# DJT777/xlstm-yolo-clean

Hardware: NVIDIA B200
Metric: mLSTM chunkwise fwd+bwd TFLOP/s (algorithmic, 14*L*d*(L+d) per chunk) (higher is better)
Workload: dtype bf16

## Files before the change

### xlstm_yolo_clean_b200/csrc/tensor_kernels.cu

```cuda
#include <atomic>
#include <mutex>
#include <set>
#include <type_traits>
#include <utility>

#include "common.cuh"
#include "sm100.cuh"

namespace mlstm {
namespace {

using namespace sm100;

constexpr int LT = 128;
constexpr int kWorkers = 256;
constexpr int kTcThreads = 320;
constexpr int kCtlWarp = 8, kScanWarp = 9;
constexpr int kNbAB = kWorkers + 32;
constexpr int kNbC = kWorkers + 64;
constexpr float kLog2e = 1.4426950408889634f;
enum { NB_A = 1, NB_B = 2, NB_C = 3, NB_PAIR0 = 4 };

struct GateBuf {
  static constexpr int oB = 0, oI = LT, oPm = 2 * LT, oY = 3 * LT, oF = 4 * LT, oMt = 5 * LT, oNt = 6 * LT,
// ... 1041 lines not shown
        for (int u = ch; u < 4; u += 2) {
          float v[32];
          const bool off_diag = REV ? u > rb : u < rb;
          if (off_diag) {
            tmem_ld32(tS + lane_base + u * 32, v);
            const float r_t = ex2_approx(x_t + gb[GateBuf::oScal + 4 + u]);
#pragma unroll
            for (int j4 = 0; j4 < 8; ++j4) {
              const float4 cf = *reinterpret_cast<const float4*>(scf + u * 32 + 4 * j4);
              v[4 * j4 + 0] *= cf.x * r_t;
              v[4 * j4 + 1] *= cf.y * r_t;
              v[4 * j4 + 2] *= cf.z * r_t;
              v[4 * j4 + 3] *= cf.w * r_t;
              rs += (v[4 * j4 + 0] + v[4 * j4 + 1]) + (v[4 * j4 + 2] + v[4 * j4 + 3]);
            }
          } else if (u == rb) {
            tmem_ld32(tS + lane_base + u * 32, v);
#pragma unroll
            for (int j4 = 0; j4 < 8; ++j4) {
              const float4 y = *reinterpret_cast<const float4*>(sy + u * 32 + 4 * j4);
              const float yy[4] = {y.x, y.y, y.z, y.w};
#pragma unroll
              for (int e = 0; e < 4; ++e) {
                const int j = 4 * j4 + e;
                float pv = v[j] * ex2_approx(x_t + yy[e]);
                pv = (REV ? j >= lane : j <= lane) ? pv : 0.f;
                rs += pv;
                v[j] = pv;
              }
            }
          } else {
#pragma unroll
            for (int j = 0; j < 32; ++j) v[j] = 0.f;
          }
          store_row32<T>(sP, row, u * 32, v);
        }
        srs[ch * LT + row] = rs;
      }
      fence_proxy_async_smem();
      tc_fence_before_sync();
      named_arrive(NB_B, kNbAB);
      {
        const float ab = __expf(g - b_t + i_t - m_next);
#pragma unroll 1
        for (int hf = 0; hf < 2; ++hf) {
          float kb[32];
#pragma unroll
          for (int j = 0; j < 4; ++j) {
            uint4 u = *reinterpret_cast<const uint4*>(sK + ch * SM::kTile + swz128(row, hf * 32 + 8 * j));
            float2 a0 = unpack2<T>(u.x), a1 = unpack2<T>(u.y), a2 = unpack2<T>(u.z), a3 = unpack2<T>(u.w);
            kb[8 * j + 0] = a0.x * ab; kb[8 * j + 1] = a0.y * ab; kb[8 * j + 2] = a1.x * ab; kb[8 * j + 3] = a1.y * ab;
            kb[8 * j + 4] = a2.x * ab; kb[8 * j + 5] = a2.y * ab; kb[8 * j + 6] = a3.x * ab; kb[8 * j + 7] = a3.y * ab;
          }
          store_row32<T>(sKb, row, ch * 64 + hf * 32, kb);
          const float cs = warp_colsum32(kb, lane);
          snp[rb * D + ch * 64 + hf * 32 + lane] = cs;
        }
        fence_proxy_async_smem();
        named_arrive(NB_A, kNbAB);
      }
      mbar_wait(&bar_h, par, 7);
      tc_fence_after_sync();
      {
        const float bq = __expf(b_t + m_run - m_t) * p.scale;
        const float den = bq * (sqn[row] + sqn[LT + row]) + srs[row] + srs[LT + row];
        const float nmax = fmaxf(fabsf(den), __expf(-m_t));
        const float inv = p.sig == 2 ? 1.f : 1.f / (nmax + p.eps);
#pragma unroll 1
        for (int hf = 0; hf < 2; ++hf) {
          uint32_t hi[32], hx[32];
          tmem_ld32_nowait(tHi + lane_base + ch * 64 + hf * 32, hi);
          tmem_ld32_nowait(tHx + lane_base + ch * 64 + hf * 32, hx);
          tmem_ld_wait();
          float o[32];
#pragma unroll
          for (int j = 0; j < 32; ++j) o[j] = (__uint_as_float(hi[j]) + bq * __uint_as_float(hx[j])) * inv;
          store_row32<T>(sH, row, ch * 64 + hf * 32, o);
        }
        if (ch == 0 && row < n_valid) {
          p.n_out[(int64_t)bh * p.S + t0 + row] = nmax;
          p.m_out[(int64_t)bh * p.S + t0 + row] = m_t;
        }
        if (EPI) {
          uint8_t* sub = sH + ch * SM::kTile;
          const int64_t tok = (int64_t)(t0 + row);
          if (p.h_plain && row < n_valid) {
            uint4* dst = reinterpret_cast<uint4*>((T*)p.h_plain + b * p.h_sb + hh * p.h_sh + tok * p.h_ss + ch * 64);
#pragma unroll
            for (int j = 0; j < 8; ++j) dst[j] = *reinterpret_cast<const uint4*>(sub + swz128(row, 8 * j));
          }
          const void* xrow = p.x ? (const void*)((const uint16_t*)p.x + b * p.x_sb + hh * p.x_sh + tok * p.x_ss + ch * 64) : nullptr;
          ln_epilogue_slice<T, 128, 64>(sub, [](int r, int cc) { return swz128(r, cc & 63); }, row, ch * 64, ch, NB_PAIR0 + rb,
                                        fsm + SM::fStat, fsm + SM::fPar, xrow, p.xy_f16 != 0, p.ln_eps, row < n_valid);
        }
      }
      mbar_wait(&bar_dc, par, 6);
      tc_fence_after_sync();
      {
#pragma unroll
        for (int hf = 0; hf < 2; ++hf) {
          float v[32], t32[32];
          tmem_ld32(tDC + lane_base + ch * 64 + hf * 32, v);
#pragma unroll
          for (int j = 0; j < 32; ++j) {
            Creg[hf * 32 + j] = gbar * Creg[hf * 32 + j] + v[j];
            t32[j] = Creg[hf * 32 + j];
          }
          store_row32<T>(sC, row, ch * 64 + hf * 32, t32);
        }
        if (tid < D) {
          sNn[tid] = gbar * sNc[tid] + ((snp[tid] + snp[D + tid]) + (snp[2 * D + tid] + snp[3 * D + tid]));
          mbar_arrive(&bar_n);
        }
      }
      fence_proxy_async_smem();
      tc_fence_before_sync();
      named_arrive(NB_C, kNbC);
      m_run = m_next;
      cur ^= 1;
    }
    if (p.c_last) {
      float* dst = p.c_last + ((int64_t)bh * D + row) * D + ch * 64;
#pragma unroll
      for (int j = 0; j < 64; ++j) dst[j] = Creg[j];
      if (tid < D) p.n_last[(int64_t)bh * D + tid] = fsm[SM::fN + cur * D + tid];
      if (tid == 0) p.m_last[bh] = m_run;
    }
  }
  tc_fence_before_sync();
  __syncthreads();
  if (warp == kCtlWarp) tmem_dealloc<512>(tmem);
}

struct TcBwParams {
  int B, NH, S, NT;
  float eps, scale;
  const void *ig, *fg;
  int64_t ig_sb, ig_sh, ig_ss, fg_sb, fg_sh, fg_ss;
  const float* m0;
  const float *n_out, *m_out, *dc_last;
  void *di, *df;
  int64_t di_sb, di_sh, di_ss, df_sb, df_sh, df_ss;
  float* dc0;
  int rev;
  int sig;
  float cap;
  int acc_qk, acc_v, acc_g;
  int cs_rows, cs_off;
#ifdef MLSTM_TC_PROFILE
  long long* prof;
#endif
};

template <int D_>
struct BwSmem {
  static constexpr int D = D_;
  static constexpr int kTile = Lay<D>::kTile;
  static constexpr int kPTile = LT * 128;
  static constexpr int kState = Lay<D>::kState;
  static constexpr int kNST = D == 64 ? 1 : 2;
  static constexpr int kStage = 4 * kTile + kState;
  static constexpr int oQ = 0, oK = kTile, oV = 2 * kTile, odH = 3 * kTile, oCs = 4 * kTile;
  static constexpr int oQt = kNST * kStage;
  static constexpr int oSb = oQt + kTile;
  static constexpr int odS = oSb + 2 * kPTile;
  static constexpr int odQ = odS + 2 * kPTile;
  static constexpr int odV = odQ + kTile;
  static constexpr int odK = odV + kTile;
  static constexpr int odC = odK + kTile;
  static constexpr int oSmall = odC + kState;
  static constexpr int fGates = 0, fPart = 2 * GateBuf::kFloats, kSmallFloats = fPart + 12 * LT;
  static constexpr int kBytes = oSmall + kSmallFloats * 4 + 1024;
  static constexpr uint32_t kLoadBytes = 4 * kTile + kState;
  static constexpr bool kAlias = D == 64;
  static constexpr uint32_t cS = 0, cdSb = 128;
  static constexpr uint32_t cdV1 = D == 64 ? 0 : 256, cdV2 = cdV1 + D, cdK1 = D == 64 ? 128 : 320, cdK2 = cdK1 + D,
                            cdQa = D == 64 ? 256 : 384, cdQb = cdQa + D, cddC = D == 64 ? 384 : 448;
};

template <typename T, int D, bool REV, typename TO>
__global__ void __launch_bounds__(kTcThreads, 1)
tc_bw(const __grid_constant__ CUtensorMap mapQ, const __grid_constant__ CUtensorMap mapK,
          const __grid_constant__ CUtensorMap mapV, const __grid_constant__ CUtensorMap mapdH,
          const __grid_constant__ CUtensorMap mapCs, const __grid_constant__ CUtensorMap mapdQ,
          const __grid_constant__ CUtensorMap mapdK, const __grid_constant__ CUtensorMap mapdV, TcBwParams p) {
  constexpr bool kBf16 = std::is_same<T, __nv_bfloat16>::value;
  using SM = BwSmem<D>;
  using L = Lay<D>;
  constexpr int CW = L::CW;
  TC_PROF(200, 0);
  TC_PROF_CTA(0);
  extern __shared__ uint8_t smem_raw[];
  uint8_t* smem = smem_raw + ((1024u - (smem_u32(smem_raw) & 1023u)) & 1023u);
  uint8_t* sQ = smem + SM::oQ;
  uint8_t* sK = smem + SM::oK;
  uint8_t* sV = smem + SM::oV;
  uint8_t* sdH = smem + SM::odH;
  uint8_t* sQt = smem + SM::oQt;
  uint8_t* sSb = smem + SM::oSb;
  uint8_t* sdS = smem + SM::odS;
  uint8_t* sdQ = smem + SM::odQ;
  uint8_t* sdV = smem + SM::odV;
  uint8_t* sdK = smem + SM::odK;
  uint8_t* sCs = smem + SM::oCs;
  uint8_t* sdC = smem + SM::odC;
  float* fsm = (float*)(smem + SM::oSmall);
  __shared__ uint64_t bar_full[SM::kNST], bar_s, bar_q, bar_v, bar_k, bar_d, bar_b, bar_st, bar_g[2];
  __shared__ uint32_t tmem_base_s;

  const int tid = threadIdx.x, lane = tid & 31;
  const int warp = __shfl_sync(0xffffffffu, tid >> 5, 0);
  const int bh = blockIdx.x, b = bh / p.NH, hh = bh % p.NH;

  auto mt = [&](int c) { return REV ? p.NT - 1 - c : c; };
  auto load_stage = [&](int s, int c) {
    uint8_t* base = smem + s * SM::kStage;
    mbar_expect_tx(&bar_full[s], SM::kLoadBytes);
    tma_load_4d(base + SM::oQ, &mapQ, &bar_full[s], 0, mt(c) * LT, hh, b);
    tma_load_4d(base + SM::oK, &mapK, &bar_full[s], 0, mt(c) * LT, hh, b);
    tma_load_4d(base + SM::oV, &mapV, &bar_full[s], 0, mt(c) * LT, hh, b);
    tma_load_4d(base + SM::odH, &mapdH, &bar_full[s], 0, mt(c) * LT, hh, b);
    tma_load_4d(base + SM::oCs, &mapCs, &bar_full[s], 0, mt(c) * p.cs_rows + p.cs_off, hh, b);
  };
  if (tid == kCtlWarp * 32) {
    for (int s = 0; s < SM::kNST; ++s) mbar_init(&bar_full[s], 1);
    fence_mbar_init();
    grid_dep_wait();
    for (int s = 0; s < SM::kNST && s < p.NT; ++s) load_stage(s, p.NT - 1 - s);
  }
  if (tid == 0) {
    mbar_init(&bar_s, 1);
    mbar_init(&bar_b, 1);
    mbar_init(&bar_st, 1);
    mbar_init(&bar_q, 1);
    mbar_init(&bar_v, 1);
    mbar_init(&bar_k, 1);
    mbar_init(&bar_d, 1);
    mbar_init(&bar_g[0], 1);
    mbar_init(&bar_g[1], 1);
    fence_mbar_init();
  }
  if (warp == kCtlWarp) {
    tmem_alloc<512>(&tmem_base_s);
    if (lane == 0) {
      prefetch_tmap(&mapQ); prefetch_tmap(&mapK); prefetch_tmap(&mapV); prefetch_tmap(&mapdH);
      prefetch_tmap(&mapCs); prefetch_tmap(&mapdQ); prefetch_tmap(&mapdK); prefetch_tmap(&mapdV);
    }
  }
  grid_dep_wait();
  grid_dep_launch();
  const int rb = warp & 3, ch = (warp >> 2) & 1;
  const int row = rb * 32 + lane;
  const uint32_t lane_base = (uint32_t)(rb * 32) << 16;
  const int drow = rb * 16 + (lane & 15);
  const bool owns_c = warp < kCtlWarp && lane < 16 && rb * 16 < D;
  float dCreg[CW];
#pragma unroll
  for (int j = 0; j < CW; ++j) dCreg[j] = 0.f;
  if (warp < kCtlWarp) {
    if (p.dc_last && owns_c) {
      const float* src = p.dc_last + ((int64_t)bh * D + drow) * D + ch * CW;
#pragma unroll
      for (int j = 0; j < CW; ++j) dCreg[j] = src[j];
    }
    if (owns_c) store_cols<T, D>(sdC, drow, ch * CW, dCreg);
    fence_proxy_async_smem();
  }
  tc_fence_before_sync();
  __syncthreads();
  tc_fence_after_sync();
  const uint32_t tmem = tmem_base_s;
  const uint32_t tS = tmem + SM::cS, tdSb = tmem + SM::cdSb;
  const uint32_t tdV1 = tmem + SM::cdV1, tdV2 = tmem + SM::cdV2, tdK1 = tmem + SM::cdK1, tdK2 = tmem + SM::cdK2;
  const uint32_t tdQa = tmem + SM::cdQa, tdQb = tmem + SM::cdQb, tddC = tmem + SM::cddC;

  const T* ip = (const T*)p.ig + b * p.ig_sb + hh * p.ig_sh;
  const T* fp = (const T*)p.fg + b * p.fg_sb + hh * p.fg_sh;
  const float* mo = p.m_out + (int64_t)bh * p.S;
  const float* no = p.n_out + (int64_t)bh * p.S;
  if (warp == kCtlWarp) {
    constexpr uint32_t id_s = umma_idesc(128, 128, false, false, kBf16);
    constexpr uint32_t id_c = umma_idesc(64, D, true, true, kBf16);
    constexpr uint32_t id_k_mn = umma_idesc(128, D, false, true, kBf16);
    constexpr uint32_t id_mn_mn = umma_idesc(128, D, true, true, kBf16);
    constexpr uint32_t id_k_k = umma_idesc(128, D, false, false, kBf16);
    const uint64_t kQ0 = L::desc(smem_u32(sQ), 0), mQ0 = L::desc(smem_u32(sQ), SM::kTile);
    const uint64_t kK0 = L::desc(smem_u32(sK), 0), mK0 = L::desc(smem_u32(sK), SM::kTile);
    const uint64_t kV0 = L::desc(smem_u32(sV), 0);
    const uint64_t kH0 = L::desc(smem_u32(sdH), 0), mH0 = L::desc(smem_u32(sdH), SM::kTile);
    const uint64_t kCs0 = L::desc(smem_u32(sCs), 0);
    const uint64_t mQt = L::desc(smem_u32(sQt), D == 64 ? SM::kTile : 0);
    const uint64_t mSb = umma_smem_desc(smem_u32(sSb), SM::kPTile, 1024);
    const uint64_t kdS = umma_smem_desc(smem_u32(sdS), 0, 1024), mdS = umma_smem_desc(smem_u32(sdS), SM::kPTile, 1024);
    const uint64_t kdC = L::desc(smem_u32(sdC), 0), mdC = L::desc(smem_u32(sdC), SM::kState);
    auto issue_s = [&](int it) {
      const int s = it % SM::kNST;
      const uint32_t so = (uint32_t)s * SM::kStage;
      const uint64_t kQ = umma_desc_advance(kQ0, so), kK = umma_desc_advance(kK0, so);
      const uint64_t kH = umma_desc_advance(kH0, so), kV = umma_desc_advance(kV0, so);
      mbar_wait(&bar_full[s], (it / SM::kNST) & 1, 11);
      tc_fence_after_sync();
#pragma unroll
      for (int kk = 0; kk < D / 16; ++kk)
        umma_f16(tS, umma_desc_advance(kQ, kk * 32), umma_desc_advance(kK, kk * 32), id_s, kk > 0);
#pragma unroll
      for (int kk = 0; kk < D / 16; ++kk)
        umma_f16(tdSb, umma_desc_advance(kH, kk * 32), umma_desc_advance(kV, kk * 32), id_s, kk > 0);
      umma_commit(&bar_s);
    };

    if (elect_one()) issue_s(0);
    __syncwarp();

    for (int it = 0; it < p.NT; ++it) {
      const int c = p.NT - 1 - it, pb = it & 1;
      const uint32_t par = it & 1;
      const int t0 = mt(c) * LT, n_valid = min(LT, p.S - t0);
      const uint32_t so = (uint32_t)(it % SM::kNST) * SM::kStage;
      const uint64_t kQ = umma_desc_advance(kQ0, so), mQ = umma_desc_advance(mQ0, so);
      const uint64_t kK = umma_desc_advance(kK0, so), mK = umma_desc_advance(mK0, so);
      const uint64_t kV = umma_desc_advance(kV0, so), kCs = umma_desc_advance(kCs0, so);
      const uint64_t kH = umma_desc_advance(kH0, so), mH = umma_desc_advance(mH0, so);
      TC_PROF(it, 9);
      if (SM::kNST == 1 && c > 0 && lane == 0) {
        const int r = mt(c - 1) * LT;
        tma_prefetch_4d(&mapQ, 0, r, hh, b);
        tma_prefetch_4d(&mapK, 0, r, hh, b);
        tma_prefetch_4d(&mapV, 0, r, hh, b);
        tma_prefetch_4d(&mapdH, 0, r, hh, b);
        tma_prefetch_4d(&mapCs, 0, mt(c - 1) * p.cs_rows + p.cs_off, hh, b);
      }
      named_sync(NB_B, kNbAB);
      TC_PROF(it, 10);
      if (elect_one()) {
        tc_fence_after_sync();
#pragma unroll
        for (int kk = 0; kk < LT / 16; ++kk)
          umma_f16(tdK1, umma_desc_advance(mdS, kk * 2048), umma_desc_advance(mQ, kk * L::kAdvMN), id_mn_mn, kk > 0);
#pragma unroll
        for (int kk = 0; kk < D / 16; ++kk)
          umma_f16(tdK2, umma_desc_advance(kV, kk * 32), umma_desc_advance(kdC, kk * 32), id_k_k, kk > 0);
        umma_commit(&bar_k);
#pragma unroll
        for (int kk = 0; kk < LT / 16; ++kk)
          umma_f16(tdQa, umma_desc_advance(kdS, (kk / 4) * SM::kPTile + (kk % 4) * 32), umma_desc_advance(mK, kk * L::kAdvMN),
                   id_k_mn, kk > 0);
#pragma unroll
        for (int kk = 0; kk < D / 16; ++kk)
          umma_f16(tdQb, umma_desc_advance(kH, kk * 32), umma_desc_advance(kCs, kk * 32), id_k_k, kk > 0);
        umma_commit(&bar_q);
#pragma unroll
        for (int kk = 0; kk < D / 16; ++kk)
          umma_f16(tdV2, umma_desc_advance(kK, kk * 32), umma_desc_advance(mdC, kk * L::kAdvMN), id_k_mn, kk > 0);
        umma_commit(&bar_b);
      }
      __syncwarp();
      if (lane == 0) {
        tma_store_wait_read<0>();
        mbar_arrive(&bar_st);
      }
      __syncwarp();
      TC_PROF(it, 11);
      named_sync(NB_A, kNbAB);
      TC_PROF(it, 12);
      if (elect_one()) {
#pragma unroll
        for (int kk = 0; kk < LT / 16; ++kk)
          umma_f16(tddC, umma_desc_advance(mQt, kk * L::kAdvMN), umma_desc_advance(mH, kk * L::kAdvMN), id_c, kk > 0);
        umma_commit(&bar_d);
#pragma unroll
        for (int kk = 0; kk < LT / 16; ++kk)
          umma_f16(tdV1, umma_desc_advance(mSb, kk * 2048), umma_desc_advance(mH, kk * L::kAdvMN), id_mn_mn, kk > 0);
        umma_commit(&bar_v);
        if (!SM::kAlias && c > 0) issue_s(it + 1);
        if (SM::kNST == 1) {
          if (c > 0) {
            const int r = mt(c - 1) * LT;
            mbar_expect_tx(&bar_full[0], SM::kLoadBytes);
            mbar_wait(&bar_k, par, 21);
            tma_load_4d(sQ, &mapQ, &bar_full[0], 0, r, hh, b);
            tma_load_4d(sV, &mapV, &bar_full[0], 0, r, hh, b);
            mbar_wait(&bar_q, par, 24);
            tma_load_4d(sCs, &mapCs, &bar_full[0], 0, mt(c - 1) * p.cs_rows + p.cs_off, hh, b);
            mbar_wait(&bar_b, par, 22);
            tma_load_4d(sK, &mapK, &bar_full[0], 0, r, hh, b);
            mbar_wait(&bar_v, par, 25);
            tma_load_4d(sdH, &mapdH, &bar_full[0], 0, r, hh, b);
          }
        } else if (c >= SM::kNST) {
          mbar_wait(&bar_v, par, 25);
          load_stage(it % SM::kNST, c - SM::kNST);
        }
      }
      __syncwarp();
      TC_PROF(it, 13);
      named_sync(NB_C, kNbC);
      TC_PROF(it, 14);
      if (lane == 0) {
        if (p.acc_qk) {
          tma_reduce_add_4d(&mapdQ, sdQ, 0, t0, hh, b);
          tma_reduce_add_4d(&mapdK, sdK, 0, t0, hh, b);
        } else {
          tma_store_4d(&mapdQ, sdQ, 0, t0, hh, b);
          tma_store_4d(&mapdK, sdK, 0, t0, hh, b);
        }
        if (p.acc_v) tma_reduce_add_4d(&mapdV, sdV, 0, t0, hh, b);
        else tma_store_4d(&mapdV, sdV, 0, t0, hh, b);
        tma_store_commit();
      }
      __syncwarp();
      if (SM::kAlias && c > 0 && elect_one()) issue_s(it + 1);
      __syncwarp();
    }
    if (lane == 0) tma_store_wait_all<0>();
  } else if (warp == kScanWarp) {
    struct TileRaw {
      GateRaw<T> g;
      float4 mt, nt;
      float m_prev, m_next;
    };
    auto raw_of = [&](int c) {
      TileRaw r;
      const int t0 = mt(c) * LT, n_valid = min(LT, p.S - t0);
      r.g = load_gate_raw<T>(ip + (int64_t)t0 * p.ig_ss, p.ig_ss, fp + (int64_t)t0 * p.fg_ss, p.fg_ss, n_valid);
      if (lane * 4 < n_valid) {
        r.mt = *reinterpret_cast<const float4*>(mo + t0 + lane * 4);
        r.nt = p.sig == 2 ? make_float4(1.f, 1.f, 1.f, 1.f) : *reinterpret_cast<const float4*>(no + t0 + lane * 4);
      } else {
        r.mt = make_float4(0.f, 0.f, 0.f, 0.f);
        r.nt = make_float4(1.f, 1.f, 1.f, 1.f);
      }
      if (!REV) {
        r.m_prev = c > 0 ? mo[t0 - 1] : (p.m0 ? p.m0[bh] : 0.f);
        r.m_next = mo[t0 + n_valid - 1];
      } else {
        r.m_prev = c > 0 ? mo[t0 + LT] : (p.m0 ? p.m0[bh] : 0.f);
        r.m_next = mo[t0];
      }
      return r;
    };
    auto publish = [&](float* gb, const TileRaw& r) {
      gate_scan_regs(gb, r.g, REV, p.sig != 0, p.cap);
      reinterpret_cast<float4*>(gb + GateBuf::oMt)[lane] = r.mt;
      reinterpret_cast<float4*>(gb + GateBuf::oNt)[lane] = r.nt;
      if (lane == 0) {
        gb[GateBuf::oScal + 2] = r.m_prev;
        gb[GateBuf::oScal + 3] = r.m_next;
      }
    };

    TileRaw raw = raw_of(p.NT - 1);
    float carry = 0.f;
    for (int n = 0; n < p.NT + 2; ++n) {
      if (n >= 2) {
      const int it = n - 2;
      const int c = p.NT - 1 - it, pb = it & 1;
      const int t0 = mt(c) * LT, n_valid = min(LT, p.S - t0);
      named_sync(NB_C, kNbC);
      {
        const float* sp = fsm + SM::fPart + pb * 6 * LT;
        const float* gb = fsm + SM::fGates + pb * GateBuf::kFloats;
        float acc[4], di[4];
#pragma unroll
        for (int e = 0; e < 4; ++e) {
          const int t = lane * 4 + e;
          acc[e] = (sp[0 * LT + t] + sp[1 * LT + t]) - (sp[2 * LT + t] + sp[3 * LT + t]);
          di[e] = sp[4 * LT + t] + sp[5 * LT + t];
        }
        float incl, own;
        if (!REV) {
          acc[2] += acc[3];
          acc[1] += acc[2];
          acc[0] += acc[1];
          incl = own = acc[0];
#pragma unroll
          for (int o = 1; o < 32; o <<= 1) {
            float u = __shfl_down_sync(0xffffffffu, incl, o);
            if (lane + o < 32) incl += u;
          }
        } else {
          acc[1] += acc[0];
          acc[2] += acc[1];
          acc[3] += acc[2];
          incl = own = acc[3];
#pragma unroll
          for (int o = 1; o < 32; o <<= 1) {
            float u = __shfl_up_sync(0xffffffffu, incl, o);
            if (lane >= o) incl += u;
          }
        }
        const float excl = incl - own + carry;
        TO* dip = (TO*)p.di + b * p.di_sb + hh * p.di_sh;
        TO* dfp = (TO*)p.df + b * p.df_sb + hh * p.df_sh;
#pragma unroll
        for (int e = 0; e < 4; ++e) {
          const int t = lane * 4 + e;
          if (t < n_valid) {
            const float dsig = p.sig ? 1.f - __expf(gb[GateBuf::oI + t]) : 1.f;
            float gi = di[e] * dsig * gb[GateBuf::oDi + t];
            float gf = (acc[e] + excl) * sigmoid_neg_f32(gb[GateBuf::oF + t]) * gb[GateBuf::oDf + t];
            TO* pi = dip + (int64_t)(t0 + t) * p.di_ss;
            TO* pf = dfp + (int64_t)(t0 + t) * p.df_ss;
            if (p.acc_g) {
              gi += to_f32<TO>(*pi);
              gf += to_f32<TO>(*pf);
            }
            *pi = from_f32<TO>(gi);
            *pf = from_f32<TO>(gf);
          }
        }
        carry += __shfl_sync(0xffffffffu, incl, REV ? 31 : 0);
      }
      __syncwarp();
      }
      if (n < p.NT) {
        publish(fsm + SM::fGates + (n & 1) * GateBuf::kFloats, raw);
        __syncwarp();
        if (lane == 0) mbar_arrive(&bar_g[n & 1]);
        if (n + 1 < p.NT) raw = raw_of(p.NT - 2 - n);
      }
    }
  } else {
    for (int it = 0; it < p.NT; ++it) {
      const int pb = it & 1;
      const uint32_t par = it & 1;
      const float* gb = fsm + SM::fGates + pb * GateBuf::kFloats;
      float* spart = fsm + SM::fPart + pb * 6 * LT;
      const int n_valid = min(LT, p.S - mt(p.NT - 1 - it) * LT);
      const bool valid = row < n_valid;
      const uint32_t so = (uint32_t)(it % SM::kNST) * SM::kStage;

      TC_PROF(it, 0);
      mbar_wait(&bar_g[pb], (it >> 1) & 1, 12);
      const float g = gb[GateBuf::oScal], m_prev = gb[GateBuf::oScal + 2], m_next = gb[GateBuf::oScal + 3];
      const float b_t = gb[GateBuf::oB + row], i_t = gb[GateBuf::oI + row];
      const float m_t = gb[GateBuf::oMt + row], n_t = gb[GateBuf::oNt + row];
      const float rinv = !valid ? 0.f : p.sig == 2 ? 1.f : 1.f / (n_t + p.eps);
      const float bbar = valid ? __expf(b_t + m_prev - m_t) : 0.f;
      const float abar = __expf(g - b_t + i_t - m_next);
      const float gbar = __expf(g + m_prev - m_next);
      TC_PROF(it, 1);
      mbar_wait(&bar_full[it % SM::kNST], (it / SM::kNST) & 1, 13);
      uint32_t qs[CW / 2];
      {
        const float wq = p.scale * bbar * rinv;
#pragma unroll
        for (int j = 0; j < CW / 8; ++j) {
          const uint32_t off = L::swz(row, ch * CW + 8 * j);
          uint4 u = *reinterpret_cast<const uint4*>(sQ + so + off);
          qs[4 * j] = u.x; qs[4 * j + 1] = u.y; qs[4 * j + 2] = u.z; qs[4 * j + 3] = u.w;
          float2 a0 = unpack2<T>(u.x), a1 = unpack2<T>(u.y), a2 = unpack2<T>(u.z), a3 = unpack2<T>(u.w);
          u.x = pack2<T>(a0.x * wq, a0.y * wq);
          u.y = pack2<T>(a1.x * wq, a1.y * wq);
          u.z = pack2<T>(a2.x * wq, a2.y * wq);
          u.w = pack2<T>(a3.x * wq, a3.y * wq);
          *reinterpret_cast<uint4*>(sQt + off) = u;
        }
      }
      mbar_wait(&bar_s, par, 14);
      tc_fence_after_sync();
      TC_PROF(it, 2);
      {
        const float x_t = valid ? (b_t - m_t) * kLog2e + log2f(rinv) : -INFINITY;
        const float* sy = gb + GateBuf::oY;
        const float* scf = gb + GateBuf::oCf;
#pragma unroll 1
        for (int u = ch; u < 4; u += 2) {
          float v[32], w[32];
          if (REV ? u >= rb : u <= rb) {
            uint32_t rv[32], rw[32];
            tmem_ld32_nowait(tS + lane_base + u * 32, rv);
            tmem_ld32_nowait(tdSb + lane_base + u * 32, rw);
            tmem_ld_wait();
            if (u != rb) {
              const float r_t = ex2_approx(x_t + gb[GateBuf::oScal + 4 + u]);
#pragma unroll
              for (int j4 = 0; j4 < 8; ++j4) {
                const float4 cf = *reinterpret_cast<const float4*>(scf + u * 32 + 4 * j4);
                const float cc[4] = {cf.x, cf.y, cf.z, cf.w};
#pragma unroll
                for (int e = 0; e < 4; ++e) {
                  const int j = 4 * j4 + e;
                  const float wg = cc[e] * r_t;
                  v[j] = __uint_as_float(rv[j]) * wg;
                  w[j] = __uint_as_float(rw[j]) * wg;
                }
              }
            } else {
#pragma unroll
              for (int j4 = 0; j4 < 8; ++j4) {
                const float4 y = *reinterpret_cast<const float4*>(sy + u * 32 + 4 * j4);
                const float yy[4] = {y.x, y.y, y.z, y.w};
#pragma unroll
                for (int e = 0; e < 4; ++e) {
                  const int j = 4 * j4 + e;
                  float wg = ex2_approx(x_t + yy[e]);
                  wg = (REV ? j >= lane : j <= lane) ? wg : 0.f;
                  v[j] = __uint_as_float(rv[j]) * wg;
                  w[j] = __uint_as_float(rw[j]) * wg;
                }
              }
            }
          } else {
            if (it > 0) continue;
#pragma unroll
            for (int j = 0; j < 32; ++j) { v[j] = 0.f; w[j] = 0.f; }
          }
          store_row32<T>(sSb, row, u * 32, v);
          store_row32<T>(sdS, row, u * 32, w);
        }
      }
      fence_proxy_async_smem();
      tc_fence_before_sync();
      named_arrive(NB_B, kNbAB);
      TC_PROF(it, 3);
      uint32_t ks[CW / 2], vs[CW / 2];
#pragma unroll
      for (int j = 0; j < CW / 8; ++j) {
        const uint32_t off = L::swz(row, ch * CW + 8 * j);
        uint4 uk = *reinterpret_cast<const uint4*>(sK + so + off);
        ks[4 * j] = uk.x; ks[4 * j + 1] = uk.y; ks[4 * j + 2] = uk.z; ks[4 * j + 3] = uk.w;
        uint4 uv = *reinterpret_cast<const uint4*>(sV + so + off);
        vs[4 * j] = uv.x; vs[4 * j + 1] = uv.y; vs[4 * j + 2] = uv.z; vs[4 * j + 3] = uv.w;
      }
      fence_proxy_async_smem();
      named_arrive(NB_A, kNbAB);
      TC_PROF(it, 4);
      {
        uint32_t ra[CW], rq[CW];
        float o[CW];
        float dot;
        mbar_wait(&bar_k, par, 18);
        tc_fence_after_sync();
        TC_PROF(it, 5);
        tmem_ld_nowait(tdK1 + lane_base + ch * CW, ra);
        tmem_ld_nowait(tdK2 + lane_base + ch * CW, rq);
        tmem_ld_wait();
        dot = 0.f;
#pragma unroll
        for (int j = 0; j < CW / 2; ++j) {
          o[2 * j] = p.scale * __uint_as_float(ra[2 * j]) + abar * __uint_as_float(rq[2 * j]);
          o[2 * j + 1] = p.scale * __uint_as_float(ra[2 * j + 1]) + abar * __uint_as_float(rq[2 * j + 1]);
          float2 kv = unpack2<T>(ks[j]);
          dot += kv.x * o[2 * j] + kv.y * o[2 * j + 1];
        }
        mbar_wait(&bar_st, par, 19);
        store_cols<TO, D>(sdK, row, ch * CW, o);
        spart[(1 * 2 + ch) * LT + row] = dot;
        mbar_wait(&bar_q, par, 16);
        tc_fence_after_sync();
        TC_PROF(it, 6);
        tmem_ld_nowait(tdQa + lane_base + ch * CW, ra);
        tmem_ld_nowait(tdQb + lane_base + ch * CW, rq);
        tmem_ld_wait();
        const float wb = bbar * rinv;
        dot = 0.f;
#pragma unroll
        for (int j = 0; j < CW / 2; ++j) {
          o[2 * j] = p.scale * (__uint_as_float(ra[2 * j]) + wb * __uint_as_float(rq[2 * j]));
          o[2 * j + 1] = p.scale * (__uint_as_float(ra[2 * j + 1]) + wb * __uint_as_float(rq[2 * j + 1]));
          float2 qv = unpack2<T>(qs[j]);
          dot += qv.x * o[2 * j] + qv.y * o[2 * j + 1];
        }
        store_cols<TO, D>(sdQ, row, ch * CW, o);
        spart[(0 * 2 + ch) * LT + row] = dot;
      }
      mbar_wait(&bar_d, par, 15);
      tc_fence_after_sync();
      TC_PROF(it, 7);
      {
        float v[CW];
        tmem_ld(tddC + lane_base + ch * CW, v);
        if (owns_c) {
#pragma unroll
          for (int j = 0; j < CW; ++j) dCreg[j] = gbar * dCreg[j] + v[j];
          store_cols<T, D>(sdC, drow, ch * CW, dCreg);
        }
      }
      {
        uint32_t ra[CW], rq[CW];
        float o[CW];
        float dot;
        mbar_wait(&bar_v, par, 17);
        tc_fence_after_sync();
        tmem_ld_nowait(tdV1 + lane_base + ch * CW, ra);
        tmem_ld_nowait(tdV2 + lane_base + ch * CW, rq);
        tmem_ld_wait();
        dot = 0.f;
#pragma unroll
        for (int j = 0; j < CW / 2; ++j) {
          o[2 * j] = p.scale * __uint_as_float(ra[2 * j]) + abar * __uint_as_float(rq[2 * j]);
          o[2 * j + 1] = p.scale * __uint_as_float(ra[2 * j + 1]) + abar * __uint_as_float(rq[2 * j + 1]);
          float2 vv = unpack2<T>(vs[j]);
          dot += vv.x * o[2 * j] + vv.y * o[2 * j + 1];
        }
        store_cols<TO, D>(sdV, row, ch * CW, o);
        spart[(2 * 2 + ch) * LT + row] = dot;
      }
      fence_proxy_async_smem();
      tc_fence_before_sync();
      named_arrive(NB_C, kNbC);
      TC_PROF(it, 8);
    }
    if (p.dc0 && owns_c) {
      float* dst = p.dc0 + ((int64_t)bh * D + drow) * D + ch * CW;
#pragma unroll
      for (int j = 0; j < CW; ++j) dst[j] = dCreg[j];
    }
  }
  TC_PROF(200, 1);
  tc_fence_before_sync();
  __syncthreads();
  TC_PROF(200, 2);
  TC_PROF_CTA(1);
  if (warp == kCtlWarp) tmem_dealloc<512>(tmem);
}

#ifdef MLSTM_TC_PROFILE
std::atomic<long long*> g_prof{nullptr};
#define TC_SET_PROF(p, off) (p).prof = g_prof.load() ? g_prof.load() + (off) : nullptr
#else
#define TC_SET_PROF(p, off)
#endif

int num_sms() {
  static int n = 0;
  if (!n) {
    int dev = 0;
    cudaGetDevice(&dev);
    cudaDeviceGetAttribute(&n, cudaDevAttrMultiProcessorCount, dev);
  }
  return n;
}

template <typename K>
cudaError_t ensure_smem(K kern, int bytes) {
  static std::mutex mu;
  static std::set<std::pair<const void*, int>> done;
  int dev = 0;
  cudaGetDevice(&dev);
  const std::pair<const void*, int> key(reinterpret_cast<const void*>(kern), dev);
  {
    std::lock_guard<std::mutex> g(mu);
    if (done.count(key)) return cudaSuccess;
  }
  cudaError_t e = cudaFuncSetAttribute(kern, cudaFuncAttributeMaxDynamicSharedMemorySize, bytes);
  if (e == cudaSuccess) {
    std::lock_guard<std::mutex> g(mu);
    done.insert(key);
  }
  return e;
}

int pdl_mode() {
  static int v = -1;
  if (v < 0) {
    const char* e = getenv("MLSTM_B200_PDL");
    v = e ? (e[0] - '0') : 2;
    if (v < 0 || v > 2) v = 2;
  }
  return v;
}
template <typename... KArgs, typename... Args>
cudaError_t launch_pdl(bool use_pdl, void (*kern)(KArgs...), int grid, int block, size_t smem, cudaStream_t st, Args&&... args) {
  cudaLaunchConfig_t cfg = {};
  cfg.gridDim = dim3(grid), cfg.blockDim = dim3(block), cfg.dynamicSmemBytes = smem, cfg.stream = st;
  cudaLaunchAttribute attr[1];
  attr[0].id = cudaLaunchAttributeProgrammaticStreamSerialization;
  attr[0].val.programmaticStreamSerializationAllowed = 1;
  cfg.attrs = attr, cfg.numAttrs = use_pdl ? 1 : 0;
  return cudaLaunchKernelEx(&cfg, kern, std::forward<Args>(args)...);
}

template <typename T, int D>
int launch_fw(const TcFwParams& p, const CUtensorMap& mq, const CUtensorMap& mk, const CUtensorMap& mv,
              const CUtensorMap& mh, const CUtensorMap& mcs, cudaStream_t st) {
  using SM = FwSmem<D>;
  auto kern = p.epi ? (p.rev ? tc_fw<T, D, true, true> : tc_fw<T, D, false, true>)
                    : (p.rev ? tc_fw<T, D, true, false> : tc_fw<T, D, false, false>);
  MLSTM_CUDA_CHECK(ensure_smem(kern, SM::kBytes));
  MLSTM_CUDA_CHECK(launch_pdl(pdl_mode() != 0, kern, p.B * p.NH, kTcThreads, SM::kBytes, st, mq, mk, mv, mh, mcs, p));
  count_launch();
  MLSTM_CUDA_CHECK(cudaGetLastError());
  return 0;
}

template <typename... KArgs, typename... Args>
cudaError_t launch_pair_pdl(bool use_pdl, void (*kern)(KArgs...), int grid, int block, size_t smem, cudaStream_t st,
                            Args&&... args) {
  cudaLaunchConfig_t cfg = {};
  cfg.gridDim = dim3(grid), cfg.blockDim = dim3(block), cfg.dynamicSmemBytes = smem, cfg.stream = st;
  cudaLaunchAttribute attr[2];
  attr[0].id = cudaLaunchAttributeClusterDimension;
  attr[0].val.clusterDim.x = 2, attr[0].val.clusterDim.y = 1, attr[0].val.clusterDim.z = 1;
  attr[1].id = cudaLaunchAttributeProgrammaticStreamSerialization;
  attr[1].val.programmaticStreamSerializationAllowed = 1;
  cfg.attrs = attr, cfg.numAttrs = use_pdl ? 2 : 1;
  return cudaLaunchKernelEx(&cfg, kern, std::forward<Args>(args)...);
}

template <typename T, int D>
auto fw_rect_kernel(bool epi, bool rev) {
  return epi ? (rev ? tc_fw_rect<T, D, true, true> : tc_fw_rect<T, D, false, true>)
             : (rev ? tc_fw_rect<T, D, true, false> : tc_fw_rect<T, D, false, false>);
}

template <typename T, int D>
int launch_fw_rect(const TcFwParams& p, const CUtensorMap& mq, const CUtensorMap& mk, const CUtensorMap& mv,
                   const CUtensorMap& mh, const CUtensorMap& mcs, cudaStream_t st) {
  using SM = FwSmem<D>;
  auto kern = fw_rect_kernel<T, D>(p.epi != 0, p.rev != 0);
  if (p.epi) {
    MLSTM_CUDA_CHECK(ensure_smem(kern, SM::kBytesPair));
    MLSTM_CUDA_CHECK(launch_pair_pdl(pdl_mode() != 0, kern, 2 * p.B * p.NH, kTcThreads, SM::kBytesPair, st, mq, mk, mv, mh, mcs, p));
  } else {
    MLSTM_CUDA_CHECK(ensure_smem(kern, SM::kBytes));
    MLSTM_CUDA_CHECK(launch_pdl(pdl_mode() != 0, kern, 2 * p.B * p.NH, kTcThreads, SM::kBytes, st, mq, mk, mv, mh, mcs, p));
  }
  count_launch();
  MLSTM_CUDA_CHECK(cudaGetLastError());
  return 0;
}

template <typename T>
int launch_fw_d128(const TcFwParams& p, const CUtensorMap& mq, const CUtensorMap& mk, const CUtensorMap& mv,
                   const CUtensorMap& mh, const CUtensorMap& mcs, cudaStream_t st) {
  auto kern = p.epi ? (p.rev ? tc_fw_d128<T, true, true> : tc_fw_d128<T, false, true>)
                    : (p.rev ? tc_fw_d128<T, true, false> : tc_fw_d128<T, false, false>);
  MLSTM_CUDA_CHECK(ensure_smem(kern, FwSmem128::kBytes));
  kern<<<p.B * p.NH, kTcThreads, FwSmem128::kBytes, st>>>(mq, mk, mv, mh, mcs, p);
  count_launch();
  MLSTM_CUDA_CHECK(cudaGetLastError());
  return 0;
}

template <typename T, int D, typename TO = T>
int launch_bw(const TcBwParams& p, const CUtensorMap& mq, const CUtensorMap& mk, const CUtensorMap& mv,
              const CUtensorMap& mdh, const CUtensorMap& mcs, const CUtensorMap& mdq, const CUtensorMap& mdk,
              const CUtensorMap& mdv, cudaStream_t st) {
  using SM = BwSmem<D>;
  auto kern = p.rev ? tc_bw<T, D, true, TO> : tc_bw<T, D, false, TO>;
  MLSTM_CUDA_CHECK(ensure_smem(kern, SM::kBytes));
  MLSTM_CUDA_CHECK(launch_pdl(pdl_mode() == 1, kern, p.B * p.NH, kTcThreads, SM::kBytes, st, mq, mk, mv, mdh, mcs, mdq, mdk, mdv, p));
  MLSTM_CUDA_CHECK(cudaGetLastError());
  return 0;
}

bool tma_ok(const mlstm_b200_tensor& t) {
  return ((uintptr_t)t.ptr & 15) == 0 && t.stride[3] == 1 && (t.stride[0] % 8) == 0 && (t.stride[1] % 8) == 0 &&
         (t.stride[2] % 8) == 0;
}

int make_map(CUtensorMap* m, const mlstm_b200_tensor& t, const mlstm_b200_shape& s, int D, int box = 0) {
  return sm100_host::make_map_bhsd(m, t.ptr, s.dtype == MLSTM_B200_BF16, s.B, s.NH, s.S, D, t.stride[0], t.stride[1],
                                   t.stride[2], LT, box ? box : D == 32 ? 32 : 64);
}
int make_states_map(CUtensorMap* m, const void* ptr, const mlstm_b200_shape& s) {
  const int NT = (s.S + LT - 1) / LT, D = s.DHQK;
  return sm100_host::make_map_bhsd(m, ptr, s.dtype == MLSTM_B200_BF16, s.B, s.NH, NT * D, D, (int64_t)s.NH * NT * D * D,
                                   (int64_t)NT * D * D, D, D, D);
// ... 357 lines not shown
```

Measured before the change: 250.5.

## Merge dV accumulators into one TMEM tile and split Q/K barrier for D=64

For the D=64 bf16 backward kernel, the two dV matmuls (intra-chunk and state term) are folded into one TMEM accumulator. The folding pre-scales the gate weights per row and keeps dC in a rescaled fixed range (2^-64), so a single MMA chain accumulates both terms. Q/K loads get their own mbarrier and the S and dS MMAs are issued separately, so S can start before V/dH/Cs arrive and the S and dS epilogues overlap. The scaling and max-clamp trick adds numerical risk and more barrier logic in exchange for fewer TMEM loads and MMAs and earlier MMA issue.

```diff
diff --git a/xlstm_yolo_clean_b200/csrc/tensor_kernels.cu b/xlstm_yolo_clean_b200/csrc/tensor_kernels.cu
--- a/xlstm_yolo_clean_b200/csrc/tensor_kernels.cu
+++ b/xlstm_yolo_clean_b200/csrc/tensor_kernels.cu
@@ -1217,7 +1217,7 @@
 #endif
 };
 
-template <int D_>
+template <int D_, bool MERGE = false>
 struct BwSmem {
   static constexpr int D = D_;
   static constexpr int kTile = Lay<D>::kTile;
@@ -1234,13 +1234,17 @@
   static constexpr int odK = odV + kTile;
   static constexpr int odC = odK + kTile;
   static constexpr int oSmall = odC + kState;
-  static constexpr int fGates = 0, fPart = 2 * GateBuf::kFloats, kSmallFloats = fPart + 12 * LT;
+  static constexpr int fGates = 0, fPart = 2 * GateBuf::kFloats, fGv = fPart + 12 * LT, kSmallFloats = fGv + 2 * LT;
   static constexpr int kBytes = oSmall + kSmallFloats * 4 + 1024;
   static constexpr uint32_t kLoadBytes = 4 * kTile + kState;
-  static constexpr bool kAlias = D == 64;
+  static constexpr uint32_t kLoadBytesQK = 2 * kTile;
+  static constexpr bool kMerge = MERGE;
+  static_assert(!MERGE || D == 64, "the merged dV accumulator is laid out for D = 64");
   static constexpr uint32_t cS = 0, cdSb = 128;
-  static constexpr uint32_t cdV1 = D == 64 ? 0 : 256, cdV2 = cdV1 + D, cdK1 = D == 64 ? 128 : 320, cdK2 = cdK1 + D,
-                            cdQa = D == 64 ? 256 : 384, cdQb = cdQa + D, cddC = D == 64 ? 384 : 448;
+  static constexpr uint32_t cdV1 = MERGE ? 448 : D == 64 ? 0 : 256, cdV2 = MERGE ? cdV1 : cdV1 + D,
+                            cdK1 = D == 64 ? 128 : 320, cdK2 = cdK1 + D, cdQa = D == 64 ? 256 : 384, cdQb = cdQa + D,
+                            cddC = D == 64 ? 384 : 448;
+  static_assert(kBytes + 256  <= 227 * 1024, "shared memory per CTA");
 };
 
 template <typename T, int D, bool REV, typename TO>
@@ -1250,7 +1254,7 @@
           const __grid_constant__ CUtensorMap mapCs, const __grid_constant__ CUtensorMap mapdQ,
           const __grid_constant__ CUtensorMap mapdK, const __grid_constant__ CUtensorMap mapdV, TcBwParams p) {
   constexpr bool kBf16 = std::is_same<T, __nv_bfloat16>::value;
-  using SM = BwSmem<D>;
+  using SM = BwSmem<D, D == 64 && kBf16>;
   using L = Lay<D>;
   constexpr int CW = L::CW;
   TC_PROF(200, 0);
@@ -1270,7 +1274,7 @@
   uint8_t* sCs = smem + SM::oCs;
   uint8_t* sdC = smem + SM::odC;
   float* fsm = (float*)(smem + SM::oSmall);
-  __shared__ uint64_t bar_full[SM::kNST], bar_s, bar_q, bar_v, bar_k, bar_d, bar_b, bar_st, bar_g[2];
+  __shared__ uint64_t bar_full[SM::kNST], bar_qk, bar_s, bar_ds, bar_kr, bar_q, bar_v, bar_k, bar_d, bar_b, bar_st, bar_g[2];
   __shared__ uint32_t tmem_base_s;
 
   const int tid = threadIdx.x, lane = tid & 31;
@@ -1280,21 +1284,26 @@
   auto mt = [&](int c) { return REV ? p.NT - 1 - c : c; };
   auto load_stage = [&](int s, int c) {
     uint8_t* base = smem + s * SM::kStage;
-    mbar_expect_tx(&bar_full[s], SM::kLoadBytes);
-    tma_load_4d(base + SM::oQ, &mapQ, &bar_full[s], 0, mt(c) * LT, hh, b);
-    tma_load_4d(base + SM::oK, &mapK, &bar_full[s], 0, mt(c) * LT, hh, b);
+    uint64_t* bqk = SM::kMerge ? &bar_qk : &bar_full[s];
+    if (SM::kMerge) mbar_expect_tx(&bar_qk, SM::kLoadBytesQK);
+    mbar_expect_tx(&bar_full[s], SM::kMerge ? SM::kLoadBytes - SM::kLoadBytesQK : SM::kLoadBytes);
+    tma_load_4d(base + SM::oQ, &mapQ, bqk, 0, mt(c) * LT, hh, b);
+    tma_load_4d(base + SM::oK, &mapK, bqk, 0, mt(c) * LT, hh, b);
     tma_load_4d(base + SM::oV, &mapV, &bar_full[s], 0, mt(c) * LT, hh, b);
     tma_load_4d(base + SM::odH, &mapdH, &bar_full[s], 0, mt(c) * LT, hh, b);
     tma_load_4d(base + SM::oCs, &mapCs, &bar_full[s], 0, mt(c) * p.cs_rows + p.cs_off, hh, b);
   };
   if (tid == kCtlWarp * 32) {
     for (int s = 0; s < SM::kNST; ++s) mbar_init(&bar_full[s], 1);
+    mbar_init(&bar_qk, 1);
     fence_mbar_init();
     grid_dep_wait();
     for (int s = 0; s < SM::kNST && s < p.NT; ++s) load_stage(s, p.NT - 1 - s);
   }
   if (tid == 0) {
     mbar_init(&bar_s, 1);
+    mbar_init(&bar_ds, 1);
+    mbar_init(&bar_kr, kWorkers / 32);
     mbar_init(&bar_b, 1);
     mbar_init(&bar_st, 1);
     mbar_init(&bar_q, 1);
@@ -1319,6 +1328,7 @@
   const uint32_t lane_base = (uint32_t)(rb * 32) << 16;
   const int drow = rb * 16 + (lane & 15);
   const bool owns_c = warp < kCtlWarp && lane < 16 && rb * 16 < D;
+  constexpr float kDcScale = SM::kMerge ? 0x1p-64f : 1.f;
   float dCreg[CW];
 #pragma unroll
   for (int j = 0; j < CW; ++j) dCreg[j] = 0.f;
@@ -1326,7 +1336,7 @@
     if (p.dc_last && owns_c) {
       const float* src = p.dc_last + ((int64_t)bh * D + drow) * D + ch * CW;
 #pragma unroll
-      for (int j = 0; j < CW; ++j) dCreg[j] = src[j];
+      for (int j = 0; j < CW; ++j) dCreg[j] = src[j] * kDcScale;
     }
     if (owns_c) store_cols<T, D>(sdC, drow, ch * CW, dCreg);
     fence_proxy_async_smem();
@@ -1362,19 +1372,29 @@
       const int s = it % SM::kNST;
       const uint32_t so = (uint32_t)s * SM::kStage;
       const uint64_t kQ = umma_desc_advance(kQ0, so), kK = umma_desc_advance(kK0, so);
-      const uint64_t kH = umma_desc_advance(kH0, so), kV = umma_desc_advance(kV0, so);
-      mbar_wait(&bar_full[s], (it / SM::kNST) & 1, 11);
+      mbar_wait(SM::kMerge ? &bar_qk : &bar_full[s], (it / SM::kNST) & 1, 11);
       tc_fence_after_sync();
 #pragma unroll
       for (int kk = 0; kk < D / 16; ++kk)
         umma_f16(tS, umma_desc_advance(kQ, kk * 32), umma_desc_advance(kK, kk * 32), id_s, kk > 0);
+      umma_commit(&bar_s);
+    };
+    auto issue_ds = [&](int it) {
+      const int s = it % SM::kNST;
+      const uint32_t so = (uint32_t)s * SM::kStage;
+      const uint64_t kH = umma_desc_advance(kH0, so), kV = umma_desc_advance(kV0, so);
+      if (SM::kMerge) mbar_wait(&bar_full[s], (it / SM::kNST) & 1, 27);
+      tc_fence_after_sync();
 #pragma unroll
       for (int kk = 0; kk < D / 16; ++kk)
         umma_f16(tdSb, umma_desc_advance(kH, kk * 32), umma_desc_advance(kV, kk * 32), id_s, kk > 0);
-      umma_commit(&bar_s);
+      umma_commit(&bar_ds);
     };
 
-    if (elect_one()) issue_s(0);
+    if (elect_one()) {
+      issue_s(0);
+      issue_ds(0);
+    }
     __syncwarp();
 
     for (int it = 0; it < p.NT; ++it) {
@@ -1435,22 +1455,33 @@
         umma_commit(&bar_d);
 #pragma unroll
         for (int kk = 0; kk < LT / 16; ++kk)
-          umma_f16(tdV1, umma_desc_advance(mSb, kk * 2048), umma_desc_advance(mH, kk * L::kAdvMN), id_mn_mn, kk > 0);
+          umma_f16(tdV1, umma_desc_advance(mSb, kk * 2048), umma_desc_advance(mH, kk * L::kAdvMN), id_mn_mn,
+                   SM::kMerge || kk > 0);
         umma_commit(&bar_v);
-        if (!SM::kAlias && c > 0) issue_s(it + 1);
+        if (SM::kNST == 2 && c > 0) {
+          issue_s(it + 1);
+          issue_ds(it + 1);
+        }
         if (SM::kNST == 1) {
           if (c > 0) {
             const int r = mt(c - 1) * LT;
-            mbar_expect_tx(&bar_full[0], SM::kLoadBytes);
+            uint64_t* bqk = SM::kMerge ? &bar_qk : &bar_full[0];
+            if (SM::kMerge) mbar_expect_tx(&bar_qk, SM::kLoadBytesQK);
+            mbar_expect_tx(&bar_full[0], SM::kMerge ? SM::kLoadBytes - SM::kLoadBytesQK : SM::kLoadBytes);
             mbar_wait(&bar_k, par, 21);
-            tma_load_4d(sQ, &mapQ, &bar_full[0], 0, r, hh, b);
+            tma_load_4d(sQ, &mapQ, bqk, 0, r, hh, b);
             tma_load_4d(sV, &mapV, &bar_full[0], 0, r, hh, b);
             mbar_wait(&bar_q, par, 24);
             tma_load_4d(sCs, &mapCs, &bar_full[0], 0, mt(c - 1) * p.cs_rows + p.cs_off, hh, b);
             mbar_wait(&bar_b, par, 22);
-            tma_load_4d(sK, &mapK, &bar_full[0], 0, r, hh, b);
+            tma_load_4d(sK, &mapK, bqk, 0, r, hh, b);
             mbar_wait(&bar_v, par, 25);
             tma_load_4d(sdH, &mapdH, &bar_full[0], 0, r, hh, b);
+            if (SM::kMerge) {
+              issue_s(it + 1);
+              mbar_wait(&bar_kr, par, 26);
+              issue_ds(it + 1);
+            }
           }
         } else if (c >= SM::kNST) {
           mbar_wait(&bar_v, par, 25);
@@ -1474,7 +1505,10 @@
         tma_store_commit();
       }
       __syncwarp();
-      if (SM::kAlias && c > 0 && elect_one()) issue_s(it + 1);
+      if (SM::kNST == 1 && !SM::kMerge && c > 0 && elect_one()) {
+        issue_s(it + 1);
+        issue_ds(it + 1);
+      }
       __syncwarp();
     }
     if (lane == 0) tma_store_wait_all<0>();
@@ -1504,13 +1538,29 @@
       }
       return r;
     };
-    auto publish = [&](float* gb, const TileRaw& r) {
+    auto publish = [&](float* gb, float* gv, const TileRaw& r) {
       gate_scan_regs(gb, r.g, REV, p.sig != 0, p.cap);
       reinterpret_cast<float4*>(gb + GateBuf::oMt)[lane] = r.mt;
       reinterpret_cast<float4*>(gb + GateBuf::oNt)[lane] = r.nt;
       if (lane == 0) {
         gb[GateBuf::oScal + 2] = r.m_prev;
         gb[GateBuf::oScal + 3] = r.m_next;
+      }
+      if (SM::kMerge) {
+        __syncwarp();
+        const float g = gb[GateBuf::oScal];
+        const float4 bv = reinterpret_cast<const float4*>(gb + GateBuf::oB)[lane];
+        const float4 iv = reinterpret_cast<const float4*>(gb + GateBuf::oI)[lane];
+        const float4 cf = reinterpret_cast<const float4*>(gb + GateBuf::oCf)[lane];
+        const float bb[4] = {bv.x, bv.y, bv.z, bv.w}, ii[4] = {iv.x, iv.y, iv.z, iv.w}, cc[4] = {cf.x, cf.y, cf.z, cf.w};
+        float gs[4], cs[4];
+#pragma unroll
+        for (int e = 0; e < 4; ++e) {
+          gs[e] = p.scale / fmaxf(__expf(g - bb[e] + ii[e] - r.m_next) * (1.f / kDcScale), 1.f);
+          cs[e] = cc[e] * gs[e];
+        }
+        reinterpret_cast<float4*>(gv)[lane] = make_float4(gs[0], gs[1], gs[2], gs[3]);
+        reinterpret_cast<float4*>(gb + GateBuf::oPm)[lane] = make_float4(cs[0], cs[1], cs[2], cs[3]);
       }
     };
 
@@ -1579,7 +1629,7 @@
       __syncwarp();
       }
       if (n < p.NT) {
-        publish(fsm + SM::fGates + (n & 1) * GateBuf::kFloats, raw);
+        publish(fsm + SM::fGates + (n & 1) * GateBuf::kFloats, fsm + SM::fGv + (n & 1) * LT, raw);
         __syncwarp();
         if (lane == 0) mbar_arrive(&bar_g[n & 1]);
         if (n + 1 < p.NT) raw = raw_of(p.NT - 2 - n);
@@ -1605,7 +1655,7 @@
       const float abar = __expf(g - b_t + i_t - m_next);
       const float gbar = __expf(g + m_prev - m_next);
       TC_PROF(it, 1);
-      mbar_wait(&bar_full[it % SM::kNST], (it / SM::kNST) & 1, 13);
+      mbar_wait(SM::kMerge ? &bar_qk : &bar_full[it % SM::kNST], (it / SM::kNST) & 1, 13);
       uint32_t qs[CW / 2];
       {
         const float wq = p.scale * bbar * rinv;
@@ -1629,49 +1679,84 @@
         const float x_t = valid ? (b_t - m_t) * kLog2e + log2f(rinv) : -INFINITY;
         const float* sy = gb + GateBuf::oY;
         const float* scf = gb + GateBuf::oCf;
+        const float* scv = SM::kMerge ? gb + GateBuf::oPm : scf;
+        const float* sgv = fsm + SM::fGv + pb * LT;
 #pragma unroll 1
         for (int u = ch; u < 4; u += 2) {
-          float v[32], w[32];
+          float v[32];
           if (REV ? u >= rb : u <= rb) {
-            uint32_t rv[32], rw[32];
+            uint32_t rv[32];
             tmem_ld32_nowait(tS + lane_base + u * 32, rv);
-            tmem_ld32_nowait(tdSb + lane_base + u * 32, rw);
             tmem_ld_wait();
             if (u != rb) {
               const float r_t = ex2_approx(x_t + gb[GateBuf::oScal + 4 + u]);
 #pragma unroll
               for (int j4 = 0; j4 < 8; ++j4) {
-                const float4 cf = *reinterpret_cast<const float4*>(scf + u * 32 + 4 * j4);
+                const float4 cf = *reinterpret_cast<const float4*>(scv + u * 32 + 4 * j4);
                 const float cc[4] = {cf.x, cf.y, cf.z, cf.w};
 #pragma unroll
-                for (int e = 0; e < 4; ++e) {
-                  const int j = 4 * j4 + e;
-                  const float wg = cc[e] * r_t;
-                  v[j] = __uint_as_float(rv[j]) * wg;
-                  w[j] = __uint_as_float(rw[j]) * wg;
-                }
+                for (int e = 0; e < 4; ++e) v[4 * j4 + e] = __uint_as_float(rv[4 * j4 + e]) * (cc[e] * r_t);
               }
             } else {
 #pragma unroll
               for (int j4 = 0; j4 < 8; ++j4) {
                 const float4 y = *reinterpret_cast<const float4*>(sy + u * 32 + 4 * j4);
                 const float yy[4] = {y.x, y.y, y.z, y.w};
+                float4 gvv = make_float4(1.f, 1.f, 1.f, 1.f);
+                if (SM::kMerge) gvv = *reinterpret_cast<const float4*>(sgv + u * 32 + 4 * j4);
+                const float gg[4] = {gvv.x, gvv.y, gvv.z, gvv.w};
 #pragma unroll
                 for (int e = 0; e < 4; ++e) {
                   const int j = 4 * j4 + e;
                   float wg = ex2_approx(x_t + yy[e]);
                   wg = (REV ? j >= lane : j <= lane) ? wg : 0.f;
-                  v[j] = __uint_as_float(rv[j]) * wg;
-                  w[j] = __uint_as_float(rw[j]) * wg;
+                  v[j] = __uint_as_float(rv[j]) * (SM::kMerge ? wg * gg[e] : wg);
                 }
               }
             }
           } else {
             if (it > 0) continue;
 #pragma unroll
-            for (int j = 0; j < 32; ++j) { v[j] = 0.f; w[j] = 0.f; }
+            for (int j = 0; j < 32; ++j) v[j] = 0.f;
           }
           store_row32<T>(sSb, row, u * 32, v);
+        }
+        mbar_wait(&bar_ds, par, 20);
+        tc_fence_after_sync();
+#pragma unroll 1
+        for (int u = ch; u < 4; u += 2) {
+          float w[32];
+          if (REV ? u >= rb : u <= rb) {
+            uint32_t rw[32];
+            tmem_ld32_nowait(tdSb + lane_base + u * 32, rw);
+            tmem_ld_wait();
+            if (u != rb) {
+              const float r_t = ex2_approx(x_t + gb[GateBuf::oScal + 4 + u]);
+#pragma unroll
+              for (int j4 = 0; j4 < 8; ++j4) {
+                const float4 cf = *reinterpret_cast<const float4*>(scf + u * 32 + 4 * j4);
+                const float cc[4] = {cf.x, cf.y, cf.z, cf.w};
+#pragma unroll
+                for (int e = 0; e < 4; ++e) w[4 * j4 + e] = __uint_as_float(rw[4 * j4 + e]) * (cc[e] * r_t);
+              }
+            } else {
+#pragma unroll
+              for (int j4 = 0; j4 < 8; ++j4) {
+                const float4 y = *reinterpret_cast<const float4*>(sy + u * 32 + 4 * j4);
+                const float yy[4] = {y.x, y.y, y.z, y.w};
+#pragma unroll
+                for (int e = 0; e < 4; ++e) {
+                  const int j = 4 * j4 + e;
+                  const float wg = ex2_approx(x_t + yy[e]);
+                  w[j] = __uint_as_float(rw[j]) * ((REV ? j >= lane : j <= lane) ? wg : 0.f);
+                }
+              }
+            }
+          } else {
+            if (it > 0) continue;
+#pragma unroll
+            for (int j = 0; j < 32; ++j) w[j] = 0.f;
+          }
           store_row32<T>(sdS, row, u * 32, w);
         }
       }
@@ -1680,6 +1765,7 @@
       named_arrive(NB_B, kNbAB);
       TC_PROF(it, 3);
       uint32_t ks[CW / 2], vs[CW / 2];
+      if (SM::kMerge) mbar_wait(&bar_full[0], par, 13);
 #pragma unroll
       for (int j = 0; j < CW / 8; ++j) {
         const uint32_t off = L::swz(row, ch * CW + 8 * j);
@@ -1701,11 +1787,17 @@
         tmem_ld_nowait(tdK1 + lane_base + ch * CW, ra);
         tmem_ld_nowait(tdK2 + lane_base + ch * CW, rq);
         tmem_ld_wait();
+        if (SM::kMerge) {
+          tc_fence_before_sync();
+          __syncwarp();
+          if (lane == 0) mbar_arrive(&bar_kr);
+        }
+        const float abk = abar * (1.f / kDcScale);
         dot = 0.f;
 #pragma unroll
         for (int j = 0; j < CW / 2; ++j) {
-          o[2 * j] = p.scale * __uint_as_float(ra[2 * j]) + abar * __uint_as_float(rq[2 * j]);
-          o[2 * j + 1] = p.scale * __uint_as_float(ra[2 * j + 1]) + abar * __uint_as_float(rq[2 * j + 1]);
+          o[2 * j] = p.scale * __uint_as_float(ra[2 * j]) + abk * __uint_as_float(rq[2 * j]);
+          o[2 * j + 1] = p.scale * __uint_as_float(ra[2 * j + 1]) + abk * __uint_as_float(rq[2 * j + 1]);
           float2 kv = unpack2<T>(ks[j]);
           dot += kv.x * o[2 * j] + kv.y * o[2 * j + 1];
         }
@@ -1738,24 +1830,32 @@
         tmem_ld(tddC + lane_base + ch * CW, v);
         if (owns_c) {
 #pragma unroll
-          for (int j = 0; j < CW; ++j) dCreg[j] = gbar * dCreg[j] + v[j];
+          for (int j = 0; j < CW; ++j) dCreg[j] = gbar * dCreg[j] + v[j] * kDcScale;
           store_cols<T, D>(sdC, drow, ch * CW, dCreg);
         }
       }
       {
-        uint32_t ra[CW], rq[CW];
+        uint32_t ra[CW];
         float o[CW];
         float dot;
         mbar_wait(&bar_v, par, 17);
         tc_fence_after_sync();
         tmem_ld_nowait(tdV1 + lane_base + ch * CW, ra);
-        tmem_ld_nowait(tdV2 + lane_base + ch * CW, rq);
-        tmem_ld_wait();
+        if constexpr (SM::kMerge) {
+          tmem_ld_wait();
+          const float F = fmaxf(abar * (1.f / kDcScale), 1.f);
+#pragma unroll
+          for (int j = 0; j < CW; ++j) o[j] = F * __uint_as_float(ra[j]);
+        } else {
+          uint32_t rq[CW];
+          tmem_ld_nowait(tdV2 + lane_base + ch * CW, rq);
+          tmem_ld_wait();
+#pragma unroll
+          for (int j = 0; j < CW; ++j) o[j] = p.scale * __uint_as_float(ra[j]) + abar * __uint_as_float(rq[j]);
+        }
         dot = 0.f;
 #pragma unroll
         for (int j = 0; j < CW / 2; ++j) {
-          o[2 * j] = p.scale * __uint_as_float(ra[2 * j]) + abar * __uint_as_float(rq[2 * j]);
-          o[2 * j + 1] = p.scale * __uint_as_float(ra[2 * j + 1]) + abar * __uint_as_float(rq[2 * j + 1]);
           float2 vv = unpack2<T>(vs[j]);
           dot += vv.x * o[2 * j] + vv.y * o[2 * j + 1];
         }
@@ -1770,7 +1870,7 @@
     if (p.dc0 && owns_c) {
       float* dst = p.dc0 + ((int64_t)bh * D + drow) * D + ch * CW;
 #pragma unroll
-      for (int j = 0; j < CW; ++j) dst[j] = dCreg[j];
+      for (int j = 0; j < CW; ++j) dst[j] = dCreg[j] * (1.f / kDcScale);
     }
   }
   TC_PROF(200, 1);
```

Result: slower. 232.2, median of 6 (-7.3%).
